# stanFurrer/Robust-Multimodal-Contrastive-Learning

Hardware: AMD Instinct MI355X
Metric: image-text pairs/sec, ViLT-B/32 RMCL step (PGD K=3) (higher is better)
Workload: dtype bf16; 1 GPU; RMCL step, PGD K=3 image attack + MoCo InfoNCE (queue 65536) + full backward + AdamW, ViLT-B/32, bs=64/GPU, 384x384 img + 40 tok (BASELINE configs[2]; [3] when n_gpus=8); global_batch=64, parallelism=dp1, grad_sync=ring/f32, ln_fold=on (shift-robust form)

## Files before the change

robust-multimodal-contrastive-learning_amd/csrc/api.cpp:

```cpp
#include "rmcl_common.h"
#include "kernels.h"
#include "../../include/rmcl.h"
#include <mutex>
#include <string>
#include <unordered_set>

static thread_local std::string g_err;
extern "C" void rmcl_set_error(const char* msg) { g_err = msg ? msg : ""; }

int rmcl_attention_fwd_impl(const void* qkv, const int* mask, void* out, void* probs, float* scores, int B, int N, int H, int dt,
                            int exact, hipStream_t s);
int rmcl_attention_bwd_impl(const void* qkv, const int* mask, const void* probs, const void* dout, const void* out, void* dqkv,
                            float* scores, void* dS, int B, int N, int H, int dt, int exact, hipStream_t s);

#include <vector>
namespace {
struct Prof {
  bool on = false;
  int mask = 0;
  size_t n = 0, cap = 0;
  std::vector<hipEvent_t> ev;
  double flops = 0.0;
} g_prof;
}
// ... 67 lines not shown
  double ms = 0.0;
  for (size_t i = 0; i < g_prof.n; ++i) {
    float t = 0.f;
    HIP_TRY(hipEventSynchronize(g_prof.ev[2 * i + 1]));
    HIP_TRY(hipEventElapsedTime(&t, g_prof.ev[2 * i], g_prof.ev[2 * i + 1]));
    ms += t;
  }
  if (ms_total) *ms_total = ms;
  if (launches) *launches = (int64_t)g_prof.n;
  if (flops_total) *flops_total = g_prof.flops;
  return 0;
}
int rmcl_version(void) { return 1; }

int rmcl_dropout_mask_apply(float* x, int64_t n, uint32_t drop_seed, int layer, int site, float drop_p, void* stream) {
  RMCL_REQUIRE(x && drop_p >= 0.f && drop_p < 1.f, "dropout_mask_apply: bad argument");
  if (drop_p == 0.f) return 0;
  return rmcl_dropout_apply(x, n, rmcl_site_seed(drop_seed, layer, site), (uint32_t)((double)drop_p * 4294967296.0), 1.0f / (1.0f - drop_p),
                            (hipStream_t)stream);
}
extern int g_st_reserve_cus;
extern bool g_attn_fused_bwd;
extern bool g_dw_grouped;
extern int g_attn_fwd_waves;
extern int g_infonce_fold;
extern int g_dp_stagger;
extern int g_attn_bwd_persist;
extern int g_attn_bwd_tpw;
extern int g_gemm_share;
extern bool g_lnfold_centred;
extern int g_prefetch_mask, g_prefetch_wgs;
extern int g_st_res_lds;
extern bool g_preact_tiled;
int rmcl_l2_prefetch_experiment(const void* A, int64_t lda_bytes, int M, int rows_per_tile, int tiles_per_xcd, int col_tiles, const void* B,
                                int64_t ldb_bytes, int nB, int nk, int tick, int lead, int per_xcd, int wgs, int* counter, int64_t* stamps, void* stream) {
  RMCL_REQUIRE(A && B && counter && M > 0 && nk > 0 && per_xcd > 0 && wgs > 0 && col_tiles > 0, "l2_prefetch_experiment: bad argument");
  return rmcl_debug_l2_prefetch(A, (long)lda_bytes, M, rows_per_tile, tiles_per_xcd, col_tiles, B, (long)ldb_bytes, nB, nk, tick, lead, per_xcd, wgs, counter,
                                reinterpret_cast<long long*>(stamps), (hipStream_t)stream);
}
int rmcl_tune_set(int key, int value) {
  if (key == 11) { g_lnfold_centred = value != 0; return 0; }
  if (key == 12) { g_prefetch_mask = value & 7; return 0; }
  if (key == 13) { g_prefetch_wgs = value < 0 ? 0 : (value > 64 ? 64 : value); return 0; }
  if (key == 15) { g_preact_tiled = value != 0; return 0; }
  if (key == 14) { g_st_res_lds = value != 0; return 0; }
  if (key == 7) { g_dp_stagger = value < 0 ? 0 : value; return 0; }
  if (key == 10) { g_gemm_share = value < 1 ? 1 : (value > 8 ? 8 : value); return 0; }
  if (key == 9) { g_attn_bwd_tpw = value; return 0; }
  if (key == 8) { g_attn_bwd_persist = value < 0 ? 0 : value; return 0; }
  if (key == 6) { rmcl_gemm_skinny_set_form(value); return 0; }
  if (key == 0) { rmcl_gemm_fast_set_cfg(value); return 0; }
  if (key == 1) { g_st_reserve_cus = value < 0 ? 0 : (value > 128 ? 128 : value); return 0; }
  if (key == 2) { g_attn_fused_bwd = value != 0; return 0; }
  if (key == 5) { g_infonce_fold = value != 0; return 0; }
  if (key == 4) { g_attn_fwd_waves = value; return 0; }
  if (key == 3) { g_dw_grouped = value != 0; return 0; }
  rmcl_set_error("tune_set: unknown key");
  return -1;
}

int64_t rmcl_heads_stash_bytes(const rmcl_dims* d) { return (int64_t)carve_heads(*d, nullptr, nullptr) + 256; }

int rmcl_heads_forward(const rmcl_dims* d, const float* pool32, const float* head32, const float* xn, void* hstash,
                       float* cls_feats, float* q, void* stream) {
  return rmcl_heads_forward2(d, pool32, head32, xn, hstash, cls_feats, q, 0, stream);
}
int rmcl_heads_forward2(const rmcl_dims* d, const float* pool32, const float* head32, const float* xn, void* hstash,
                        float* cls_feats, float* q, int flags, void* stream) {
  RMCL_REQUIRE(d && pool32 && xn && hstash && cls_feats, "heads_forward: NULL argument");
  RMCL_REQUIRE((flags & ~RMCL_HEADS_NO_WGRAD) == 0, "heads_forward: unknown flag");
  rmcl_layout y;
  rmcl_param_layout(d, &y);
  HeadStash h;
// ... 386 lines not shown
```

robust-multimodal-contrastive-learning_amd/csrc/gemm_sw.hip:

```cpp
#include <type_traits>
#include "rmcl_common.h"
#include "kernels.h"

typedef __bf16 bf16x8 __attribute__((ext_vector_type(8)));
typedef __attribute__((address_space(3))) void lds_void;
typedef const __attribute__((address_space(1))) void glb_void;

#define SW_UNIT 24576
#define SW_BUF (3 * SW_UNIT)
#define SW_LDS (2 * SW_BUF)


#ifdef ST_TRACE
__device__ long long g_sw_trace[2][32];
#define SW_STAMP(i)                                                                                              \
  if (blockIdx.x == 100 && (threadIdx.x & 255) == 0) g_sw_trace[threadIdx.x >> 8][i] = wall_clock64()
extern "C" int rmcl_debug_sw_trace(long long* out) {
  return (int)hipMemcpyFromSymbol(out, HIP_SYMBOL(g_sw_trace), sizeof(long long) * 64);
}
#else
#define SW_STAMP(i)
#endif

template <int N>
__device__ __forceinline__ void sw_wait_vm() {
  asm volatile("s_waitcnt vmcnt(%0)" ::"n"(N) : "memory");
}

__device__ __forceinline__ void sw_stage(const bf16_t* base, const uint32_t (&off)[3], long koff, char* lds_unit, int wave) {
#pragma unroll
  for (int q = 0; q < 3; ++q)
    __builtin_amdgcn_global_load_lds((glb_void*)(base + koff + off[q]), (lds_void*)(lds_unit + (wave * 3 + q) * 1024), 16, 0, 0);
}

__device__ __forceinline__ int sw_gk(int k) { return ((k >> 1) & 1) | (((k >> 3) & 1) << 1); }

template <bool KC>
__device__ __forceinline__ bf16x8 sw_ld(const char* unit, int off, int s) {
  if (KC) {
    return *reinterpret_cast<const bf16x8*>(unit + off);
  } else {
    union { bf16x8 v; s16x4 h[2]; } u;
#pragma unroll
    for (int h = 0; h < 2; ++h)
      u.h[h] = __builtin_amdgcn_ds_read_tr16_b64_v4i16((__attribute__((address_space(3))) s16x4*)(unit + off + s * (32 * 384) + h * (4 * 384)));
    return u.v;
  }
}

#define SW_PHASE_BEGIN()                                  \
  __builtin_amdgcn_sched_barrier(0);                      \
  __builtin_amdgcn_s_barrier();                           \
  asm volatile("s_waitcnt lgkmcnt(0)" ::: "memory");      \
  __builtin_amdgcn_sched_barrier(0);                      \
  __builtin_amdgcn_s_setprio(1)
#define SW_PHASE_END()                                    \
  __builtin_amdgcn_s_setprio(0);                          \
  __builtin_amdgcn_sched_barrier(0);                      \
  __builtin_amdgcn_s_barrier();                           \
  __builtin_amdgcn_sched_barrier(0)

enum { SW_AUX_NONE = 0, SW_AUX_RES = 1, SW_AUX_DGELU = 2, SW_AUX_DGELU_T = 3, SW_AUX_STASH_T = 4 };

struct SWCtx {
  const bf16_t* A;
  const bf16_t* B;
  uint32_t oa[3], ob0[3], ob1[3];
  int aoff[2], boff[2], boffj[3];
  long kstep_b;
  int wave;
};

struct SWAux {
  const bf16_t* aux;
  long ld;
  int m0, n0, M;
};
__device__ __forceinline__ void sw_stage_aux(const SWAux& x, int ch, int unit, char* area, int wave, int lane) {
#pragma unroll
  for (int q = 0; q < 3; ++q) {
    const int L = unit * SW_UNIT + (wave * 3 + q) * 1024 + lane * 16;
    const int r = L / 768, p = (L - r * 768) >> 4;
    const int trow = (r / 48) * 96 + ch * 48 + (r % 48);
    const long m = min(x.m0 + trow, x.M - 1);
    const bf16_t* src = x.aux + m * x.ld + x.n0 + ((p ^ (r & 7)) << 3);
    __builtin_amdgcn_global_load_lds((glb_void*)src, (lds_void*)(area + unit * SW_UNIT + (wave * 3 + q) * 1024), 16, 0, 0);
  }
}

struct SWNoHook { __device__ __forceinline__ void operator()() const {} };
template <bool B_KC, bool LAST, bool AUXST = false, typename HOOK = SWNoHook>
__device__ __forceinline__ void sw_ktile(f32x4 (&acc)[6][6], const SWCtx& c, const char* cur, char* oth, int t1, const SWAux* ax = nullptr, int lane = 0,
                                         const HOOK& hook = HOOK()) {
  bf16x8 a[3][2], b[3][2];
#pragma unroll
  for (int j = 0; j < 3; ++j)
#pragma unroll
    for (int s = 0; s < 2; ++s) b[j][s] = B_KC ? sw_ld<true>(cur + SW_UNIT, j * 2048 + c.boff[s], s) : sw_ld<false>(cur + SW_UNIT, c.boffj[j], s);
#pragma unroll
  for (int i = 0; i < 3; ++i)
#pragma unroll
    for (int s = 0; s < 2; ++s) a[i][s] = sw_ld<true>(cur, i * 2048 + c.aoff[s], s);
  if (!LAST) { sw_stage(c.A, c.oa, (long)t1 * 64, oth, c.wave); sw_wait_vm<3>(); } else { sw_wait_vm<0>(); if (AUXST) sw_stage_aux(*ax, 0, 0, oth, c.wave, lane); hook(); }
  SW_PHASE_BEGIN();
#pragma unroll
  for (int s = 0; s < 2; ++s)
#pragma unroll
    for (int i = 0; i < 3; ++i)
#pragma unroll
      for (int j = 0; j < 3; ++j) acc[i][j] = __builtin_amdgcn_mfma_f32_16x16x32_bf16(b[j][s], a[i][s], acc[i][j], 0, 0, 0);
  SW_PHASE_END();
#pragma unroll
  for (int j = 0; j < 3; ++j)
#pragma unroll
    for (int s = 0; s < 2; ++s) b[j][s] = B_KC ? sw_ld<true>(cur + 2 * SW_UNIT, j * 2048 + c.boff[s], s) : sw_ld<false>(cur + 2 * SW_UNIT, c.boffj[j], s);
  if (!LAST) sw_stage(c.B, c.ob0, (long)t1 * c.kstep_b, oth + SW_UNIT, c.wave);
  else if (AUXST) sw_stage_aux(*ax, 0, 1, oth, c.wave, lane);
  SW_PHASE_BEGIN();
#pragma unroll
  for (int s = 0; s < 2; ++s)
#pragma unroll
    for (int i = 0; i < 3; ++i)
#pragma unroll
      for (int j = 0; j < 3; ++j) acc[i][3 + j] = __builtin_amdgcn_mfma_f32_16x16x32_bf16(b[j][s], a[i][s], acc[i][3 + j], 0, 0, 0);
  SW_PHASE_END();
#pragma unroll
  for (int i = 0; i < 3; ++i)
#pragma unroll
    for (int s = 0; s < 2; ++s) a[i][s] = sw_ld<true>(cur, (3 + i) * 2048 + c.aoff[s], s);
  if (!LAST) sw_stage(c.B, c.ob1, (long)t1 * c.kstep_b, oth + 2 * SW_UNIT, c.wave);
  else if (AUXST) sw_stage_aux(*ax, 0, 2, oth, c.wave, lane);
  SW_PHASE_BEGIN();
#pragma unroll
  for (int s = 0; s < 2; ++s)
#pragma unroll
    for (int i = 0; i < 3; ++i)
#pragma unroll
      for (int j = 0; j < 3; ++j) acc[3 + i][3 + j] = __builtin_amdgcn_mfma_f32_16x16x32_bf16(b[j][s], a[i][s], acc[3 + i][3 + j], 0, 0, 0);
  SW_PHASE_END();
#pragma unroll
  for (int j = 0; j < 3; ++j)
#pragma unroll
    for (int s = 0; s < 2; ++s) b[j][s] = B_KC ? sw_ld<true>(cur + SW_UNIT, j * 2048 + c.boff[s], s) : sw_ld<false>(cur + SW_UNIT, c.boffj[j], s);
  if (!LAST) sw_wait_vm<3>();
  SW_PHASE_BEGIN();
#pragma unroll
  for (int s = 0; s < 2; ++s)
#pragma unroll
    for (int i = 0; i < 3; ++i)
#pragma unroll
      for (int j = 0; j < 3; ++j) acc[3 + i][j] = __builtin_amdgcn_mfma_f32_16x16x32_bf16(b[j][s], a[i][s], acc[3 + i][j], 0, 0, 0);
  SW_PHASE_END();
}

template <bool B_KC, int AUX, typename TO, int LNF = 0, bool DROP = false>
__global__ __launch_bounds__(512) void gemm_sw_kernel(GemmArgs g, int tiles_m, int tiles_n, int rows_per_tile) {
  extern __shared__ __attribute__((aligned(16))) char smem[];
  const int t = threadIdx.x, lane = t & 63;
  const int wave = __builtin_amdgcn_readfirstlane(t >> 6);
  const int wm = wave >> 2, wn = wave & 3;
  SW_STAMP(0);
  const int nwg = tiles_m * tiles_n;
  int bid = blockIdx.x;
  {
    const int xcd = bid & 7, q = nwg >> 3, r = nwg & 7;
    bid = (xcd < r ? xcd * (q + 1) : r * (q + 1) + (xcd - r) * q) + (bid >> 3);
  }
  int tr, tc;
  if (tiles_n % 4 == 0) {
    const int band = bid / (tiles_m * 4), rem = bid - band * (tiles_m * 4);
    tr = rem >> 2;
    tc = band * 4 + (rem & 3);
  } else {
    tr = bid / tiles_n;
    tc = bid - tr * tiles_n;
  }
  const int m0 = tr * rows_per_tile, n0 = tc * 384;
  const int m_end = min(g.M, m0 + rows_per_tile);
  const int nk = g.K / 64;

  SWCtx c;
  c.A = reinterpret_cast<const bf16_t*>(g.A);
  c.B = reinterpret_cast<const bf16_t*>(g.B);
  c.wave = wave;
  c.kstep_b = B_KC ? 64 : 64 * g.ldb;
#pragma unroll
  for (int q = 0; q < 3; ++q) {
    const int row = (wave * 3 + q) * 8 + (lane >> 3);
    const int chunk = (lane & 7) ^ (row & 7);
    const int lin = (wave * 3 + q) * 64 + lane;
    const int k = lin / 24, c16 = (lin - k * 24) ^ (sw_gk(k) << 1);
    c.oa[q] = (uint32_t)min(m0 + row, g.M - 1) * (uint32_t)g.lda + chunk * 8;
    if (B_KC) {
      c.ob0[q] = (uint32_t)(n0 + row) * (uint32_t)g.ldb + chunk * 8;
      c.ob1[q] = (uint32_t)(n0 + 192 + row) * (uint32_t)g.ldb + chunk * 8;
    } else {
      c.ob0[q] = (uint32_t)k * (uint32_t)g.ldb + n0 + c16 * 8;
      c.ob1[q] = c.ob0[q] + 192;
    }
  }
#pragma unroll
  for (int s = 0; s < 2; ++s) {
    const int sw = ((4 * s + (lane >> 4)) ^ (lane & 7)) * 16;
    c.aoff[s] = (wm * 96 + (lane & 15)) * 128 + sw;
    c.boff[s] = (wn * 48 + (lane & 15)) * 128 + sw;
  }
#pragma unroll
  for (int j = 0; j < 3; ++j) {
    const int q = (lane & 15) >> 2, p = lane & 3;
    const int k = 8 * (lane >> 4) + q;
    const int c8 = (wn * 48 + j * 16) / 4 + p;
    c.boffj[j] = k * 384 + (((c8 >> 1) ^ (sw_gk(k) << 1)) * 16) + (c8 & 1) * 8;
  }

  f32x4 acc[6][6];
#pragma unroll
  for (int i = 0; i < 6; ++i)
#pragma unroll
    for (int j = 0; j < 6; ++j) acc[i][j] = f32x4{0.f, 0.f, 0.f, 0.f};

  char* buf0 = smem;
  char* buf1 = smem + SW_BUF;
  float4 pst[LNF == 1 ? 8 : 1];
  float cen = 0.f;
  if constexpr (LNF == 1) {
    if (t < 192) {
      if (n0 == 0 && g.ln_mean && g.ln_center) cen = g.ln_center[min((long)m0 + t, (long)g.M - 1)];
      const float4* pp = reinterpret_cast<const float4*>(g.ln_part + min((long)m0 + t, (long)g.M - 1) * (long)(g.ln_nparts * 2));
      if (g.ln_nparts == 16) {
#pragma unroll
        for (int q = 0; q < 8; ++q) pst[q] = pp[q];
      }
    }
  }
  sw_stage(c.A, c.oa, 0, buf0, wave);
  sw_stage(c.B, c.ob0, 0, buf0 + SW_UNIT, wave);
  sw_stage(c.B, c.ob1, 0, buf0 + 2 * SW_UNIT, wave);
  if constexpr (LNF == 1) {
    if (t < 192) {
      const long m = min((long)m0 + t, (long)g.M - 1);
      float s1 = 0.f, s2 = 0.f;
      if (g.ln_nparts == 16) {
#pragma unroll
        for (int q = 0; q < 8; ++q) { s1 += pst[q].x + pst[q].z; s2 += pst[q].y + pst[q].w; }
      } else {
        const float4* pp = reinterpret_cast<const float4*>(g.ln_part + m * (long)(g.ln_nparts * 2));
        for (int q = 0; q < g.ln_nparts / 2; ++q) { const float4 v = pp[q]; s1 += v.x + v.z; s2 += v.y + v.w; }
      }
      const float inv = 1.0f / (float)g.ln_cols, mean = s1 * inv;
      const float rstd = rsqrtf(fmaxf(s2 * inv - mean * mean, 0.f) + g.ln_eps);
      float* rowstat0 = reinterpret_cast<float*>(smem + SW_LDS);
      rowstat0[2 * t] = mean;
      rowstat0[2 * t + 1] = rstd;
      if (n0 == 0 && g.ln_mean && m0 + t < m_end) { g.ln_mean[m] = mean + cen; g.ln_rstd[m] = rstd; }
    }
    asm volatile("s_waitcnt lgkmcnt(0)" ::: "memory");
  }
  sw_wait_vm<0>();
  __builtin_amdgcn_s_barrier();
  __builtin_amdgcn_sched_barrier(0);
  if (wm == 1) __builtin_amdgcn_s_barrier();
  __builtin_amdgcn_sched_barrier(0);

  SW_STAMP(1);
  int it = 0;
  for (; it + 1 < nk; ++it) {
    char* cur = (it & 1) ? buf1 : buf0;
    char* oth = (it & 1) ? buf0 : buf1;
    sw_ktile<B_KC, false>(acc, c, cur, oth, it + 1);
  }
  constexpr bool AUX_LDS = AUX == SW_AUX_DGELU && sizeof(TO) == 2;
  constexpr bool TILED_DG = AUX == SW_AUX_DGELU_T, TILED_ST = AUX == SW_AUX_STASH_T, DG = AUX == SW_AUX_DGELU || TILED_DG;
  static_assert(!(TILED_DG || TILED_ST) || (sizeof(TO) == 2 && B_KC), "tiled stash: bf16, [cols][K] weights");
  const size_t tblk = (size_t)(tr * tiles_n + tc) * RMCL_PREACT_TILE_ELEMS + rmcl_preact_tiled_off(wave, 0, 0, 0, 0, 0);
  const int tlane = rmcl_preact_tiled_off(0, 0, 0, 0, 0, lane);
  const bf16_t* tl_in = TILED_DG ? reinterpret_cast<const bf16_t*>(g.aux) + tblk : nullptr;
  uint2 tpre[TILED_DG ? 2 : 1][3][3];
  auto tiled_load_row = [&](int GRP, int il) {
    __builtin_amdgcn_sched_barrier(0);
#pragma unroll
    for (int j = 0; j < 3; ++j)
      tpre[TILED_DG && GRP == 3 ? 1 : 0][il][j] = *reinterpret_cast<const uint2*>(tl_in + tlane + rmcl_preact_tiled_off(0, GRP >> 1, GRP & 1, il, j, 0));
    __builtin_amdgcn_sched_barrier(0);
  };
  char* last_cur = (it & 1) ? buf1 : buf0;
  char* aux_area = (it & 1) ? buf0 : buf1;
  SWAux ax{reinterpret_cast<const bf16_t*>(g.aux), (long)g.ld_aux, m0, n0, g.M};
  if constexpr (AUX_LDS) {
    sw_ktile<B_KC, true, true>(acc, c, last_cur, aux_area, 0, &ax, lane);
    sw_wait_vm<0>();
  } else if constexpr (TILED_DG) {
    auto hook = [&]() {
#pragma unroll
      for (int il = 0; il < 3; ++il) tiled_load_row(0, il);
    };
    sw_ktile<B_KC, true, false, decltype(hook)>(acc, c, last_cur, nullptr, 0, nullptr, 0, hook);
  } else {
    sw_ktile<B_KC, true>(acc, c, last_cur, nullptr, 0);
  }
  if (wm == 0) __builtin_amdgcn_s_barrier();
  if constexpr (AUX_LDS) {
    __builtin_amdgcn_s_barrier();
#pragma unroll
    for (int u = 0; u < 3; ++u) sw_stage_aux(ax, 1, u, last_cur, wave, lane);
  }

  SW_STAMP(2);
  const int epi = g.epi;
  TO* C = reinterpret_cast<TO*>(g.C);
  TO* C2 = reinterpret_cast<TO*>(g.C2);
  bf16_t* tl_out = TILED_ST ? reinterpret_cast<bf16_t*>(g.C2) + tblk : nullptr;
  const int mb = m0 + wm * 96 + (lane & 15);
  if constexpr (sizeof(TO) == 2) {
    constexpr int ROWB = 768, PIECES = 48, ROWS = 48, IMG = ROWS * ROWB;
    char* img0 = AUX_LDS ? aux_area + wm * IMG : smem + wm * (2 * IMG);
    const bool stash = !AUX_LDS && (epi & EPI_SAVE_PREACT) != 0;
    float* rowstat = reinterpret_cast<float*>(smem + SW_LDS);
    constexpr bool HOIST = !DG && !DROP;
    float4 bias2[HOIST ? 2 : 1][3], lns2[HOIST ? 2 : 1][LNF == 1 ? 3 : 1];
    if constexpr (HOIST) {
#pragma unroll
      for (int hb = 0; hb < 2; ++hb) {
        const int nbh = n0 + hb * 192 + wn * 48 + 4 * (lane >> 4);
#pragma unroll
        for (int j = 0; j < 3; ++j) {
          if constexpr (LNF == 1) {
            bias2[hb][j] = *reinterpret_cast<const float4*>(g.ln_c + nbh + j * 16);
            lns2[hb][j] = *reinterpret_cast<const float4*>(g.ln_s + nbh + j * 16);
          } else {
            bias2[hb][j] = (epi & EPI_BIAS) ? *reinterpret_cast<const float4*>(g.bias + nbh + j * 16) : make_float4(0.f, 0.f, 0.f, 0.f);
          }
        }
      }
    }
    float2 rs6[LNF == 1 ? 6 : 1];
    if constexpr (LNF == 1) {
#pragma unroll
      for (int i = 0; i < 6; ++i) rs6[i] = *reinterpret_cast<const float2*>(rowstat + 2 * (wm * 96 + i * 16 + (lane & 15)));
    }
    int woff[2][3];
#pragma unroll
    for (int hb = 0; hb < 2; ++hb)
#pragma unroll
      for (int j = 0; j < 3; ++j) {
        const int r = lane & 15, e8 = hb * 48 + wn * 12 + j * 4 + (lane >> 4);
        woff[hb][j] = r * ROWB + (((e8 >> 1) ^ (r & 7)) * 16) + (e8 & 1) * 8;
        asm volatile("" : "+v"(woff[hb][j]));
      }
    int rb_row[3], rb_lds[3];
    uint32_t rb_dst[3];
    {
      const int tg = (wave & 3) * 64 + lane, row0 = tg / PIECES, cp0 = tg - row0 * PIECES;
#pragma unroll
      for (int kk = 0; kk < 3; ++kk) {
        const int t16 = cp0 + 16 * kk, wrap = t16 >= PIECES ? 1 : 0, cp = t16 - wrap * PIECES, row = row0 + 5 * kk + wrap;
        rb_row[kk] = row;
        rb_lds[kk] = row * ROWB + cp * 16;
        rb_dst[kk] = (uint32_t)row * (uint32_t)g.ldc + (uint32_t)((cp ^ (row & 7)) * 8);
        asm volatile("" : "+v"(rb_row[kk]), "+v"(rb_lds[kk]), "+v"(rb_dst[kk]));
      }
    }
    const uint32_t dbase_aux = DROP ? (uint32_t)mb * (uint32_t)g.ld_aux : 0u, dbase_c = DROP ? (uint32_t)mb * (uint32_t)g.ldc : 0u;
    auto chunk_loop = [&](auto gelu_c, auto stash_c, auto dm_c) {
      constexpr bool GELU = decltype(gelu_c)::value, STASH = decltype(stash_c)::value;
      constexpr int DM = decltype(dm_c)::value;
#pragma unroll
      for (int ch = 0; ch < 2; ++ch) {
        char* aux_ch = ch == 0 ? aux_area : last_cur;
        char* img = AUX_LDS ? aux_ch + wm * IMG : img0;
// ... 31 lines not shown
              }
            }
          }
#pragma unroll
          for (int il = 0; il < 3; ++il) {
            const int i = ch * 3 + il;
            float mean_m = 0.f, rstd_m = 1.f;
            if constexpr (LNF == 1) { mean_m = rs6[i].x; rstd_m = rs6[i].y; }
#pragma unroll
            for (int j = 0; j < 3; ++j) {
              const f32x4 av = acc[i][hb * 3 + j], bv = f4v(bias[j]);
              f32x4 v;
              if constexpr (LNF == 1) v = rstd_m * (av - mean_m * f4v(lns[j])) + bv;
              else v = g.alpha * av + bv;
              if constexpr (TILED_DG) v *= gelu_poly_grad4(bf2f4(tpre[TILED_DG && ch * 2 + hb == 3 ? 1 : 0][il][j]));
              else if (AUX == SW_AUX_DGELU) v *= gelu_poly_grad4(bf2f4(pre[il][j]));
              if constexpr (DROP && (DM & 2) != 0) {
                if (DM == 2 || (epi & EPI_DROP_BWD)) {
                  const uint32_t di = dbase_aux + (uint32_t)(i * 16) * (uint32_t)g.ld_aux + (uint32_t)(nb + j * 16);
                  drop_scale4(g.drop_seed, di, g.drop_thresh, g.drop_inv_keep, v);
                }
              }
              const int off = woff[hb][j] + il * 16 * ROWB;
              if constexpr (STASH && TILED_ST) *reinterpret_cast<uint2*>(tl_out + tlane + rmcl_preact_tiled_off(0, ch, hb, il, j, 0)) = f2bf4(v);
              else if constexpr (STASH) *reinterpret_cast<uint2*>(img + IMG + off) = f2bf4(v);
              if constexpr (GELU) v = gelu_poly4(v);
              if constexpr (DROP && (DM & 1) != 0) {
                if (DM == 1 || (epi & EPI_DROPOUT)) {
                  const uint32_t ci = dbase_c + (uint32_t)(i * 16) * (uint32_t)g.ldc + (uint32_t)(nb + j * 16);
                  drop_scale4(g.drop_seed, ci, g.drop_thresh, g.drop_inv_keep, v);
                }
              }
              const uint2 pk = f2bf4(v);
              *reinterpret_cast<uint2*>(img + off) = pk;
            }
            if constexpr (TILED_DG) {
              if (ch * 2 + hb < 2) tiled_load_row(ch * 2 + hb + 1, il);
              if (ch * 2 + hb == 1 && il == 2) {
#pragma unroll
                for (int l3 = 0; l3 < 3; ++l3) tiled_load_row(3, l3);
              }
            }
          }
        }
        SW_STAMP(4 + 3 * ch);
        __builtin_amdgcn_s_barrier();
        {
          const int mrow = m0 + wm * 96 + ch * ROWS, lim = m_end - mrow;
          const uint32_t cbase = (uint32_t)mrow * (uint32_t)g.ldc + (uint32_t)n0;
#pragma unroll
          for (int t3 = 0; t3 < 3; ++t3)
#pragma unroll
            for (int kk = 0; kk < 3; ++kk) {
              if (rb_row[kk] + 16 * t3 < lim) {
                const size_t dst = (size_t)(cbase + (uint32_t)(16 * t3) * (uint32_t)g.ldc + rb_dst[kk]);
                *reinterpret_cast<float4*>(C + dst) = *reinterpret_cast<const float4*>(img + rb_lds[kk] + t3 * 16 * ROWB);
                if constexpr (STASH && !TILED_ST) *reinterpret_cast<float4*>(C2 + dst) = *reinterpret_cast<const float4*>(img + IMG + rb_lds[kk] + t3 * 16 * ROWB);
              }
            }
        }
        if constexpr (AUX_LDS) {
          if (ch == 0) { if (m0 + 144 <= m_end) sw_wait_vm<9>(); else sw_wait_vm<0>(); }
        }
        SW_STAMP(5 + 3 * ch);
        __builtin_amdgcn_s_barrier();
        SW_STAMP(6 + 3 * ch);
      }
    };
    {
      using T1 = std::integral_constant<bool, true>;
      using T0 = std::integral_constant<bool, false>;
      using D0 = std::integral_constant<int, 0>;
      using D1 = std::integral_constant<int, 1>;
      using D2 = std::integral_constant<int, 2>;
      using D3 = std::integral_constant<int, 3>;
      const bool gelu = (epi & EPI_GELU) != 0;
      const int dm = DROP ? (((epi & EPI_DROPOUT) ? 1 : 0) | ((epi & EPI_DROP_BWD) ? 2 : 0)) : 0;
      if constexpr (TILED_ST) {
        if constexpr (DROP) chunk_loop(T1{}, T1{}, D1{}); else chunk_loop(T1{}, T1{}, D0{});
      } else if constexpr (TILED_DG) {
        if constexpr (DROP) chunk_loop(T0{}, T0{}, D2{}); else chunk_loop(T0{}, T0{}, D0{});
      } else if constexpr (!DROP) {
        if constexpr (AUX_LDS) {
          if (gelu) chunk_loop(T1{}, T0{}, D0{}); else chunk_loop(T0{}, T0{}, D0{});
        } else {
          if (gelu && stash) chunk_loop(T1{}, T1{}, D0{});
          else if (gelu) chunk_loop(T1{}, T0{}, D0{});
          else if (stash) chunk_loop(T0{}, T1{}, D0{});
          else chunk_loop(T0{}, T0{}, D0{});
        }
      } else if constexpr (AUX_LDS) {
        if (!gelu && dm == 2) chunk_loop(T0{}, T0{}, D2{});
        else if (gelu) chunk_loop(T1{}, T0{}, D3{});
        else chunk_loop(T0{}, T0{}, D3{});
      } else {
        if (gelu && stash && dm == 1) chunk_loop(T1{}, T1{}, D1{});
        else if (gelu && !stash && dm == 1) chunk_loop(T1{}, T0{}, D1{});
        else if (gelu && stash) chunk_loop(T1{}, T1{}, D3{});
        else if (gelu) chunk_loop(T1{}, T0{}, D3{});
        else if (stash) chunk_loop(T0{}, T1{}, D3{});
        else chunk_loop(T0{}, T0{}, D3{});
      }
    }
  } else {
#pragma unroll
    for (int hb = 0; hb < 2; ++hb) {
      const int nb = n0 + hb * 192 + wn * 48 + 4 * (lane >> 4);
      float4 bias[3];
#pragma unroll
      for (int j = 0; j < 3; ++j) bias[j] = (epi & EPI_BIAS) ? *reinterpret_cast<const float4*>(g.bias + nb + j * 16) : make_float4(0.f, 0.f, 0.f, 0.f);
      uint2 pre[AUX == SW_AUX_DGELU ? 6 : 1][3];
#pragma unroll
      for (int i = 0; i < 6; ++i) {
        const long mr = min(mb + i * 16, g.M - 1);
#pragma unroll
        for (int j = 0; j < 3; ++j)
          if (AUX == SW_AUX_DGELU) pre[i][j] = *reinterpret_cast<const uint2*>(reinterpret_cast<const bf16_t*>(g.aux) + mr * g.ld_aux + nb + j * 16);
      }
#pragma unroll
      for (int i = 0; i < 6; ++i) {
        const int m = mb + i * 16;
        const bool live = m < m_end;
#pragma unroll
        for (int j = 0; j < 3; ++j) {
          const f32x4 av = acc[i][hb * 3 + j];
          float v[4] = {g.alpha * av[0] + bias[j].x, g.alpha * av[1] + bias[j].y, g.alpha * av[2] + bias[j].z, g.alpha * av[3] + bias[j].w};
          if (AUX == SW_AUX_DGELU) {
            const uint2 u = pre[i][j];
            v[0] *= gelu_poly_grad(__uint_as_float(u.x << 16)); v[1] *= gelu_poly_grad(__uint_as_float(u.x & 0xffff0000u));
            v[2] *= gelu_poly_grad(__uint_as_float(u.y << 16)); v[3] *= gelu_poly_grad(__uint_as_float(u.y & 0xffff0000u));
          }
          const long ci = (long)m * g.ldc + nb + j * 16;
          if ((epi & EPI_SAVE_PREACT) && live) store4<TO>(C2 + ci, v);
          if (epi & EPI_GELU) {
#pragma unroll
            for (int r = 0; r < 4; ++r) v[r] = gelu_poly(v[r]);
          }
          if (live) store4<TO>(C + ci, v);
        }
      }
    }
  }
#ifdef ST_TRACE
  SW_STAMP(10);
  asm volatile("s_waitcnt vmcnt(0)" ::: "memory");
  SW_STAMP(11);
#endif
}

bool rmcl_gemm_sw_supported(const GemmArgs& g, int a_kc, int b_kc) {
  if (!a_kc || g.nb1 > 1 || g.nb2 > 1 || g.splitk > 1) return false;
  if (g.N % 384 != 0 || g.K % 64 != 0 || g.K < 128) return false;
  if ((long)g.M * g.lda >= (1L << 31) || (long)(b_kc ? g.N : g.K) * g.ldb >= (1L << 31)) return false;
  if ((long)g.M * g.ldc >= (1L << 31)) return false;
  if (g.epi & ~(EPI_BIAS | EPI_GELU | EPI_SAVE_PREACT | EPI_DGELU | EPI_LNFOLD | EPI_DROPOUT | EPI_DROP_BWD | EPI_PREACT_TILED)) return false;
  if ((g.epi & EPI_DROP_BWD) && !(g.epi & EPI_DGELU)) return false;
  if ((g.epi & EPI_PREACT_TILED) && (!b_kc || !(g.epi & EPI_SAVE_PREACT) == !(g.epi & EPI_DGELU))) return false;
  if ((g.epi & EPI_PREACT_TILED) && (g.epi & EPI_SAVE_PREACT) && !(g.epi & EPI_GELU)) return false;
  if ((g.epi & EPI_PREACT_TILED) && (g.epi & EPI_DGELU) && (g.epi & (EPI_BIAS | EPI_GELU | EPI_DROPOUT))) return false;
  if (g.epi & EPI_LNFOLD) {
    if (!b_kc || (g.epi & (EPI_BIAS | EPI_DGELU)) || !g.ln_s || !g.ln_c || !g.ln_part || g.ln_nparts % 2 || g.ln_nparts <= 0 || g.ln_cols <= 0) return false;
  }
  return true;
}

double rmcl_gemm_sw_fill(const GemmArgs& g, int cus) {
  const long tiles = (long)cdiv(g.M, 192) * (g.N / 384);
  return (double)tiles / (double)(cdiv(tiles, (long)cus) * cus);
}

template <bool B_KC, int AUX, typename TO, bool DROP = false>
static int launch_sw3(const GemmArgs& g, hipStream_t s) {
  static RmclLdsOnce once;
  RMCL_TRY(rmcl_set_max_lds(once, reinterpret_cast<const void*>(gemm_sw_kernel<B_KC, AUX, TO, 0, DROP>), SW_LDS));
  const int tm = cdiv(g.M, 192), tn = g.N / 384, rows = cdiv(g.M, tm);
  RMCL_LAUNCH((gemm_sw_kernel<B_KC, AUX, TO, 0, DROP>), dim3(tm * tn), dim3(512), SW_LDS, s, g, tm, tn, rows);
  RMCL_CHECK_LAUNCH();
  return 0;
}

template <bool B_KC, int AUX>
static int launch_sw2(const GemmArgs& g, int dt_out, hipStream_t s) {
  if (g.epi & (EPI_DROPOUT | EPI_DROP_BWD)) {
    RMCL_REQUIRE(dt_out == RMCL_BF16, "gemm_sw: the dropout epilogues write bf16");
    return launch_sw3<B_KC, AUX, bf16_t, true>(g, s);
  }
  return dt_out == RMCL_F32 ? launch_sw3<B_KC, AUX, float>(g, s) : launch_sw3<B_KC, AUX, bf16_t>(g, s);
}

template <bool B_KC>
static int launch_sw(const GemmArgs& g, int dt_out, hipStream_t s) {
  if (g.epi & EPI_PREACT_TILED) {
    if constexpr (B_KC) {
      RMCL_REQUIRE(dt_out == RMCL_BF16, "gemm_sw: the tiled pre-activation stash is bf16");
      const bool drop = (g.epi & (EPI_DROPOUT | EPI_DROP_BWD)) != 0;
      if (g.epi & EPI_DGELU) return drop ? launch_sw3<true, SW_AUX_DGELU_T, bf16_t, true>(g, s) : launch_sw3<true, SW_AUX_DGELU_T, bf16_t>(g, s);
      return drop ? launch_sw3<true, SW_AUX_STASH_T, bf16_t, true>(g, s) : launch_sw3<true, SW_AUX_STASH_T, bf16_t>(g, s);
    } else {
      RMCL_REQUIRE(false, "gemm_sw: the tiled pre-activation stash needs [cols][K] weights");
    }
  }
  if (g.epi & EPI_DGELU) return launch_sw2<B_KC, SW_AUX_DGELU>(g, dt_out, s);
  return launch_sw2<B_KC, SW_AUX_NONE>(g, dt_out, s);
}

template <bool DROP, int AUX = SW_AUX_NONE>
static int launch_sw_lnf(const GemmArgs& g, hipStream_t s) {
  constexpr int LDS = SW_LDS + 2048;
  static RmclLdsOnce once;
  RMCL_TRY(rmcl_set_max_lds(once, reinterpret_cast<const void*>((gemm_sw_kernel<true, AUX, bf16_t, 1, DROP>)), LDS));
  const int tm = cdiv(g.M, 192), tn = g.N / 384, rows = cdiv(g.M, tm);
  RMCL_LAUNCH((gemm_sw_kernel<true, AUX, bf16_t, 1, DROP>), dim3(tm * tn), dim3(512), LDS, s, g, tm, tn, rows);
  RMCL_CHECK_LAUNCH();
  return 0;
}

int rmcl_launch_gemm_sw(const GemmArgs& g, int dt_out, int b_kc, hipStream_t s) {
  if (g.epi & EPI_LNFOLD) {
    RMCL_REQUIRE(b_kc && dt_out == RMCL_BF16, "gemm_sw: the LayerNorm-folded form is [rows][K] x [cols][K] with bf16 output");
    if (g.epi & EPI_PREACT_TILED) return (g.epi & EPI_DROPOUT) ? launch_sw_lnf<true, SW_AUX_STASH_T>(g, s) : launch_sw_lnf<false, SW_AUX_STASH_T>(g, s);
    return (g.epi & EPI_DROPOUT) ? launch_sw_lnf<true>(g, s) : launch_sw_lnf<false>(g, s);
  }
  return b_kc ? launch_sw<true>(g, dt_out, s) : launch_sw<false>(g, dt_out, s);
}
```

Before: 2043 pairs/s.

## Add persistent grid form to software-pipelined GEMM with next-tile prefetch

Adds a persistent variant of the 192x384 software-pipelined GEMM kernel that launches about one workgroup per CU and loops over tiles. It prefetches the next tile's A/B k-tile into LDS during the current tile's epilogue, which removes per-tile launch and ramp-up cost and tail waste when tiles exceed CUs. It is on by default whenever the tile count exceeds the CU cap, and can be turned off through a tune key. In exchange the epilogue staging image moves into the second buffer, and there are more LDS hazards and inline asm waits to keep correct.

```diff
diff --git a/robust-multimodal-contrastive-learning_amd/csrc/api.cpp b/robust-multimodal-contrastive-learning_amd/csrc/api.cpp
--- a/robust-multimodal-contrastive-learning_amd/csrc/api.cpp
+++ b/robust-multimodal-contrastive-learning_amd/csrc/api.cpp
@@ -123,6 +123,7 @@
 extern int g_prefetch_mask, g_prefetch_wgs;
 extern int g_st_res_lds;
 extern bool g_preact_tiled;
+extern int g_sw_persist;
 int rmcl_l2_prefetch_experiment(const void* A, int64_t lda_bytes, int M, int rows_per_tile, int tiles_per_xcd, int col_tiles, const void* B,
                                 int64_t ldb_bytes, int nB, int nk, int tick, int lead, int per_xcd, int wgs, int* counter, int64_t* stamps, void* stream) {
   RMCL_REQUIRE(A && B && counter && M > 0 && nk > 0 && per_xcd > 0 && wgs > 0 && col_tiles > 0, "l2_prefetch_experiment: bad argument");
@@ -130,6 +131,7 @@
                                 reinterpret_cast<long long*>(stamps), (hipStream_t)stream);
 }
 int rmcl_tune_set(int key, int value) {
+  if (key == 16) { g_sw_persist = value < 0 ? -1 : (value > 4096 ? 4096 : value); return 0; }
   if (key == 11) { g_lnfold_centred = value != 0; return 0; }
   if (key == 12) { g_prefetch_mask = value & 7; return 0; }
   if (key == 13) { g_prefetch_wgs = value < 0 ? 0 : (value > 64 ? 64 : value); return 0; }
diff --git a/robust-multimodal-contrastive-learning_amd/csrc/gemm_sw.hip b/robust-multimodal-contrastive-learning_amd/csrc/gemm_sw.hip
--- a/robust-multimodal-contrastive-learning_amd/csrc/gemm_sw.hip
+++ b/robust-multimodal-contrastive-learning_amd/csrc/gemm_sw.hip
@@ -14,7 +14,7 @@
 #ifdef ST_TRACE
 __device__ long long g_sw_trace[2][32];
 #define SW_STAMP(i)                                                                                              \
-  if (blockIdx.x == 100 && (threadIdx.x & 255) == 0) g_sw_trace[threadIdx.x >> 8][i] = wall_clock64()
+  if (blockIdx.x == 100 && (threadIdx.x & 255) == 0) g_sw_trace[threadIdx.x >> 8][(i) + sw_stamp_base] = wall_clock64()
 extern "C" int rmcl_debug_sw_trace(long long* out) {
   return (int)hipMemcpyFromSymbol(out, HIP_SYMBOL(g_sw_trace), sizeof(long long) * 64);
 }
@@ -31,6 +31,22 @@
 #pragma unroll
   for (int q = 0; q < 3; ++q)
     __builtin_amdgcn_global_load_lds((glb_void*)(base + koff + off[q]), (lds_void*)(lds_unit + (wave * 3 + q) * 1024), 16, 0, 0);
+}
+
+typedef uint32_t u32x2 __attribute__((ext_vector_type(2)));
+__device__ __forceinline__ void sw_lds_write64(uint32_t a, uint2 v) {
+  const u32x2 w = {v.x, v.y};
+  asm volatile("ds_write_b64 %0, %1" : : "v"(a), "v"(w) : "memory");
+}
+__device__ __forceinline__ f32x4 sw_lds_read128(uint32_t a) {
+  f32x4 v;
+  asm volatile("ds_read_b128 %0, %1" : "=v"(v) : "v"(a) : "memory");
+  return v;
+}
+__device__ __forceinline__ u32x2 sw_lds_read64(uint32_t a) {
+  u32x2 v;
+  asm volatile("ds_read_b64 %0, %1" : "=v"(v) : "v"(a) : "memory");
+  return v;
 }
 
 __device__ __forceinline__ int sw_gk(int k) { return ((k >> 1) & 1) | (((k >> 3) & 1) << 1); }
@@ -65,6 +81,7 @@
 struct SWCtx {
   const bf16_t* A;
   const bf16_t* B;
+  const bf16_t* B1;
   uint32_t oa[3], ob0[3], ob1[3];
   int aoff[2], boff[2], boffj[3];
   long kstep_b;
@@ -89,9 +106,9 @@
 }
 
 struct SWNoHook { __device__ __forceinline__ void operator()() const {} };
-template <bool B_KC, bool LAST, bool AUXST = false, typename HOOK = SWNoHook>
+template <bool B_KC, bool LAST, bool AUXST = false, typename HOOK = SWNoHook, bool PERS = false>
 __device__ __forceinline__ void sw_ktile(f32x4 (&acc)[6][6], const SWCtx& c, const char* cur, char* oth, int t1, const SWAux* ax = nullptr, int lane = 0,
-                                         const HOOK& hook = HOOK()) {
+                                         const HOOK& hook = HOOK(), bool nxt = false, bool nowait = false) {
   bf16x8 a[3][2], b[3][2];
 #pragma unroll
   for (int j = 0; j < 3; ++j)
@@ -101,7 +118,15 @@
   for (int i = 0; i < 3; ++i)
 #pragma unroll
     for (int s = 0; s < 2; ++s) a[i][s] = sw_ld<true>(cur, i * 2048 + c.aoff[s], s);
-  if (!LAST) { sw_stage(c.A, c.oa, (long)t1 * 64, oth, c.wave); sw_wait_vm<3>(); } else { sw_wait_vm<0>(); if (AUXST) sw_stage_aux(*ax, 0, 0, oth, c.wave, lane); hook(); }
+  if (!LAST) {
+    sw_stage(c.A, c.oa, (long)t1 * 64, oth, c.wave);
+    if (PERS) { if (!nowait) sw_wait_vm<3>(); } else sw_wait_vm<3>();
+  } else {
+    sw_wait_vm<0>();
+    if (AUXST) sw_stage_aux(*ax, 0, 0, oth, c.wave, lane);
+    hook();
+    if (PERS) { if (nxt) sw_stage(c.A, c.oa, 0, oth, c.wave); }
+  }
   SW_PHASE_BEGIN();
 #pragma unroll
   for (int s = 0; s < 2; ++s)
@@ -116,6 +141,7 @@
     for (int s = 0; s < 2; ++s) b[j][s] = B_KC ? sw_ld<true>(cur + 2 * SW_UNIT, j * 2048 + c.boff[s], s) : sw_ld<false>(cur + 2 * SW_UNIT, c.boffj[j], s);
   if (!LAST) sw_stage(c.B, c.ob0, (long)t1 * c.kstep_b, oth + SW_UNIT, c.wave);
   else if (AUXST) sw_stage_aux(*ax, 0, 1, oth, c.wave, lane);
+  else if (PERS) { if (nxt) sw_stage(c.B, c.ob0, 0, oth + SW_UNIT, c.wave); }
   SW_PHASE_BEGIN();
 #pragma unroll
   for (int s = 0; s < 2; ++s)
@@ -128,8 +154,9 @@
   for (int i = 0; i < 3; ++i)
 #pragma unroll
     for (int s = 0; s < 2; ++s) a[i][s] = sw_ld<true>(cur, (3 + i) * 2048 + c.aoff[s], s);
-  if (!LAST) sw_stage(c.B, c.ob1, (long)t1 * c.kstep_b, oth + 2 * SW_UNIT, c.wave);
+  if (!LAST) { if (PERS) sw_stage(c.B1, c.ob0, (long)t1 * c.kstep_b, oth + 2 * SW_UNIT, c.wave); else sw_stage(c.B, c.ob1, (long)t1 * c.kstep_b, oth + 2 * SW_UNIT, c.wave); }
   else if (AUXST) sw_stage_aux(*ax, 0, 2, oth, c.wave, lane);
+  else if (PERS) { if (nxt) sw_stage(c.B1, c.ob0, 0, oth + 2 * SW_UNIT, c.wave); }
   SW_PHASE_BEGIN();
 #pragma unroll
   for (int s = 0; s < 2; ++s)
@@ -153,19 +180,32 @@
   SW_PHASE_END();
 }
 
-template <bool B_KC, int AUX, typename TO, int LNF = 0, bool DROP = false>
-__global__ __launch_bounds__(512) void gemm_sw_kernel(GemmArgs g, int tiles_m, int tiles_n, int rows_per_tile) {
+template <bool B_KC, int AUX, typename TO, int LNF, bool DROP, bool PERS>
+__device__ __forceinline__ void sw_body(GemmArgs g, int tiles_m, int tiles_n, int rows_per_tile) {
+  static_assert(!PERS || (B_KC && sizeof(TO) == 2 && (AUX == SW_AUX_NONE || AUX == SW_AUX_DGELU_T || AUX == SW_AUX_STASH_T)), "persistent form: one LDS image per group");
   extern __shared__ __attribute__((aligned(16))) char smem[];
-  const int t = threadIdx.x, lane = t & 63;
+  const int t = threadIdx.x, lane0 = t & 63;
   const int wave = __builtin_amdgcn_readfirstlane(t >> 6);
   const int wm = wave >> 2, wn = wave & 3;
+  [[maybe_unused]] int sw_stamp_base = 0;
   SW_STAMP(0);
-  const int nwg = tiles_m * tiles_n;
+  const int ntiles = tiles_m * tiles_n;
+  const int nwg = PERS ? (int)gridDim.x : ntiles;
   int bid = blockIdx.x;
   {
     const int xcd = bid & 7, q = nwg >> 3, r = nwg & 7;
     bid = (xcd < r ? xcd * (q + 1) : r * (q + 1) + (xcd - r) * q) + (bid >> 3);
   }
+  auto tile_rc = [&](int id, int& r_, int& c_) {
+    if (tiles_n % 4 == 0) {
+      const int band = id / (tiles_m * 4), rem = id - band * (tiles_m * 4);
+      r_ = rem >> 2;
+      c_ = band * 4 + (rem & 3);
+    } else {
+      r_ = id / tiles_n;
+      c_ = id - r_ * tiles_n;
+    }
+  };
   int tr, tc;
   if (tiles_n % 4 == 0) {
     const int band = bid / (tiles_m * 4), rem = bid - band * (tiles_m * 4);
@@ -175,20 +215,39 @@
     tr = bid / tiles_n;
     tc = bid - tr * tiles_n;
   }
-  const int m0 = tr * rows_per_tile, n0 = tc * 384;
-  const int m_end = min(g.M, m0 + rows_per_tile);
+  int m0 = tr * rows_per_tile, n0 = tc * 384;
+  int m_end = min(g.M, m0 + rows_per_tile);
   const int nk = g.K / 64;
 
   SWCtx c;
   c.A = reinterpret_cast<const bf16_t*>(g.A);
   c.B = reinterpret_cast<const bf16_t*>(g.B);
+  c.B1 = c.B + (PERS ? (size_t)192 * (size_t)g.ldb : 0);
   c.wave = wave;
   c.kstep_b = B_KC ? 64 : 64 * g.ldb;
+  int ln = lane0;
+  auto set_offsets = [&](int m0_, int n0_) {
+#pragma unroll
+    for (int q = 0; q < 3; ++q) {
+      const int row = (wave * 3 + q) * 8 + (ln >> 3);
+      const int chunk = (ln & 7) ^ (row & 7);
+      const int lin = (wave * 3 + q) * 64 + ln;
+      const int k = lin / 24, c16 = (lin - k * 24) ^ (sw_gk(k) << 1);
+      c.oa[q] = (uint32_t)min(m0_ + row, g.M - 1) * (uint32_t)g.lda + chunk * 8;
+      if (B_KC) {
+        c.ob0[q] = (uint32_t)(n0_ + row) * (uint32_t)g.ldb + chunk * 8;
+        if (!PERS) c.ob1[q] = (uint32_t)(n0_ + 192 + row) * (uint32_t)g.ldb + chunk * 8;
+      } else {
+        c.ob0[q] = (uint32_t)k * (uint32_t)g.ldb + n0_ + c16 * 8;
+        c.ob1[q] = c.ob0[q] + 192;
+      }
+    }
+  };
 #pragma unroll
   for (int q = 0; q < 3; ++q) {
-    const int row = (wave * 3 + q) * 8 + (lane >> 3);
-    const int chunk = (lane & 7) ^ (row & 7);
-    const int lin = (wave * 3 + q) * 64 + lane;
+    const int row = (wave * 3 + q) * 8 + (lane0 >> 3);
+    const int chunk = (lane0 & 7) ^ (row & 7);
+    const int lin = (wave * 3 + q) * 64 + lane0;
     const int k = lin / 24, c16 = (lin - k * 24) ^ (sw_gk(k) << 1);
     c.oa[q] = (uint32_t)min(m0 + row, g.M - 1) * (uint32_t)g.lda + chunk * 8;
     if (B_KC) {
@@ -199,16 +258,31 @@
       c.ob1[q] = c.ob0[q] + 192;
     }
   }
+  auto set_frag_offsets = [&]() {
+#pragma unroll
+    for (int s = 0; s < 2; ++s) {
+      const int sw = ((4 * s + (ln >> 4)) ^ (ln & 7)) * 16;
+      c.aoff[s] = (wm * 96 + (ln & 15)) * 128 + sw;
+      c.boff[s] = (wn * 48 + (ln & 15)) * 128 + sw;
+    }
+#pragma unroll
+    for (int j = 0; j < 3; ++j) {
+      const int q = (ln & 15) >> 2, p = ln & 3;
+      const int k = 8 * (ln >> 4) + q;
+      const int c8 = (wn * 48 + j * 16) / 4 + p;
+      c.boffj[j] = k * 384 + (((c8 >> 1) ^ (sw_gk(k) << 1)) * 16) + (c8 & 1) * 8;
+    }
+  };
 #pragma unroll
   for (int s = 0; s < 2; ++s) {
-    const int sw = ((4 * s + (lane >> 4)) ^ (lane & 7)) * 16;
-    c.aoff[s] = (wm * 96 + (lane & 15)) * 128 + sw;
-    c.boff[s] = (wn * 48 + (lane & 15)) * 128 + sw;
+    const int sw = ((4 * s + (lane0 >> 4)) ^ (lane0 & 7)) * 16;
+    c.aoff[s] = (wm * 96 + (lane0 & 15)) * 128 + sw;
+    c.boff[s] = (wn * 48 + (lane0 & 15)) * 128 + sw;
   }
 #pragma unroll
   for (int j = 0; j < 3; ++j) {
-    const int q = (lane & 15) >> 2, p = lane & 3;
-    const int k = 8 * (lane >> 4) + q;
+    const int q = (lane0 & 15) >> 2, p = lane0 & 3;
+    const int k = 8 * (lane0 >> 4) + q;
     const int c8 = (wn * 48 + j * 16) / 4 + p;
     c.boffj[j] = k * 384 + (((c8 >> 1) ^ (sw_gk(k) << 1)) * 16) + (c8 & 1) * 8;
   }
@@ -223,7 +297,7 @@
   char* buf1 = smem + SW_BUF;
   float4 pst[LNF == 1 ? 8 : 1];
   float cen = 0.f;
-  if constexpr (LNF == 1) {
+  auto ln_fetch = [&]() {
     if (t < 192) {
       if (n0 == 0 && g.ln_mean && g.ln_center) cen = g.ln_center[min((long)m0 + t, (long)g.M - 1)];
       const float4* pp = reinterpret_cast<const float4*>(g.ln_part + min((long)m0 + t, (long)g.M - 1) * (long)(g.ln_nparts * 2));
@@ -232,15 +306,12 @@
         for (int q = 0; q < 8; ++q) pst[q] = pp[q];
       }
     }
-  }
-  sw_stage(c.A, c.oa, 0, buf0, wave);
-  sw_stage(c.B, c.ob0, 0, buf0 + SW_UNIT, wave);
-  sw_stage(c.B, c.ob1, 0, buf0 + 2 * SW_UNIT, wave);
-  if constexpr (LNF == 1) {
+  };
+  auto ln_finish = [&](auto pre_c) {
     if (t < 192) {
       const long m = min((long)m0 + t, (long)g.M - 1);
       float s1 = 0.f, s2 = 0.f;
-      if (g.ln_nparts == 16) {
+      if (decltype(pre_c)::value && g.ln_nparts == 16) {
 #pragma unroll
         for (int q = 0; q < 8; ++q) { s1 += pst[q].x + pst[q].z; s2 += pst[q].y + pst[q].w; }
       } else {
@@ -255,19 +326,47 @@
       if (n0 == 0 && g.ln_mean && m0 + t < m_end) { g.ln_mean[m] = mean + cen; g.ln_rstd[m] = rstd; }
     }
     asm volatile("s_waitcnt lgkmcnt(0)" ::: "memory");
-  }
+  };
+  if constexpr (LNF == 1) ln_fetch();
+  sw_stage(c.A, c.oa, 0, buf0, wave);
+  sw_stage(c.B, c.ob0, 0, buf0 + SW_UNIT, wave);
+  if constexpr (PERS) sw_stage(c.B1, c.ob0, 0, buf0 + 2 * SW_UNIT, wave);
+  else sw_stage(c.B, c.ob1, 0, buf0 + 2 * SW_UNIT, wave);
+  if constexpr (LNF == 1) ln_finish(std::integral_constant<bool, true>{});
   sw_wait_vm<0>();
   __builtin_amdgcn_s_barrier();
   __builtin_amdgcn_sched_barrier(0);
+  [[maybe_unused]] int tile = bid;
+  [[maybe_unused]] bool later = false;
+  for (;;) {
+  int lane = lane0;
+  if constexpr (PERS) { asm volatile("" : "+v"(lane)); ln = lane; }
   if (wm == 1) __builtin_amdgcn_s_barrier();
   __builtin_amdgcn_sched_barrier(0);
 
   SW_STAMP(1);
   int it = 0;
-  for (; it + 1 < nk; ++it) {
-    char* cur = (it & 1) ? buf1 : buf0;
-    char* oth = (it & 1) ? buf0 : buf1;
-    sw_ktile<B_KC, false>(acc, c, cur, oth, it + 1);
+  if constexpr (PERS) {
+    for (; it + 1 < nk; ++it) {
+      char* cur = (it & 1) ? buf1 : buf0;
+      char* oth = (it & 1) ? buf0 : buf1;
+      sw_ktile<B_KC, false, false, SWNoHook, true>(acc, c, cur, oth, it + 1, nullptr, 0, SWNoHook(), false, later && it == 0);
+    }
+  } else {
+    for (; it + 1 < nk; ++it) {
+      char* cur = (it & 1) ? buf1 : buf0;
+      char* oth = (it & 1) ? buf0 : buf1;
+      sw_ktile<B_KC, false>(acc, c, cur, oth, it + 1);
+    }
+  }
+  [[maybe_unused]] int ntr = tr, ntc = tc;
+  [[maybe_unused]] bool has_next = false;
+  if constexpr (PERS) {
+    has_next = tile + nwg < ntiles;
+    if (has_next) {
+      tile_rc(tile + nwg, ntr, ntc);
+      set_offsets(ntr * rows_per_tile, ntc * 384);
+    }
   }
   constexpr bool AUX_LDS = AUX == SW_AUX_DGELU && sizeof(TO) == 2;
   constexpr bool TILED_DG = AUX == SW_AUX_DGELU_T, TILED_ST = AUX == SW_AUX_STASH_T, DG = AUX == SW_AUX_DGELU || TILED_DG;
@@ -294,11 +393,21 @@
 #pragma unroll
       for (int il = 0; il < 3; ++il) tiled_load_row(0, il);
     };
-    sw_ktile<B_KC, true, false, decltype(hook)>(acc, c, last_cur, nullptr, 0, nullptr, 0, hook);
+    if constexpr (PERS) sw_ktile<B_KC, true, false, decltype(hook), true>(acc, c, last_cur, buf0, 0, nullptr, 0, hook, last_cur != buf0);
+    else sw_ktile<B_KC, true, false, decltype(hook)>(acc, c, last_cur, nullptr, 0, nullptr, 0, hook);
   } else {
-    sw_ktile<B_KC, true>(acc, c, last_cur, nullptr, 0);
+    if constexpr (PERS) sw_ktile<B_KC, true, false, SWNoHook, true>(acc, c, last_cur, buf0, 0, nullptr, 0, SWNoHook(), last_cur != buf0);
+    else sw_ktile<B_KC, true>(acc, c, last_cur, nullptr, 0);
   }
   if (wm == 0) __builtin_amdgcn_s_barrier();
+  if constexpr (PERS) {
+    if (last_cur == buf0) {
+      sw_stage(c.A, c.oa, 0, buf0, wave);
+      sw_stage(c.B, c.ob0, 0, buf0 + SW_UNIT, wave);
+      sw_stage(c.B1, c.ob0, 0, buf0 + 2 * SW_UNIT, wave);
+    }
+    __builtin_amdgcn_s_waitcnt(0xC07F);
+  }
   if constexpr (AUX_LDS) {
     __builtin_amdgcn_s_barrier();
 #pragma unroll
@@ -313,7 +422,8 @@
   const int mb = m0 + wm * 96 + (lane & 15);
   if constexpr (sizeof(TO) == 2) {
     constexpr int ROWB = 768, PIECES = 48, ROWS = 48, IMG = ROWS * ROWB;
-    char* img0 = AUX_LDS ? aux_area + wm * IMG : smem + wm * (2 * IMG);
+    char* img0 = AUX_LDS ? aux_area + wm * IMG : PERS ? buf1 + wm * IMG : smem + wm * (2 * IMG);
+    [[maybe_unused]] const uint32_t img_a = lds_addr(img0);
     const bool stash = !AUX_LDS && (epi & EPI_SAVE_PREACT) != 0;
     float* rowstat = reinterpret_cast<float*>(smem + SW_LDS);
     constexpr bool HOIST = !DG && !DROP;
@@ -334,7 +444,14 @@
       }
     }
     float2 rs6[LNF == 1 ? 6 : 1];
-    if constexpr (LNF == 1) {
+    if constexpr (LNF == 1 && PERS) {
+      u32x2 rsu[6];
+#pragma unroll
+      for (int i = 0; i < 6; ++i) rsu[i] = sw_lds_read64(lds_addr(rowstat) + 8 * (wm * 96 + i * 16 + (lane & 15)));
+      asm volatile("s_waitcnt lgkmcnt(0)" : "+v"(rsu[0]), "+v"(rsu[1]), "+v"(rsu[2]), "+v"(rsu[3]), "+v"(rsu[4]), "+v"(rsu[5]) : : "memory");
+#pragma unroll
+      for (int i = 0; i < 6; ++i) rs6[i] = make_float2(__uint_as_float(rsu[i].x), __uint_as_float(rsu[i].y));
+    } else if constexpr (LNF == 1) {
 #pragma unroll
       for (int i = 0; i < 6; ++i) rs6[i] = *reinterpret_cast<const float2*>(rowstat + 2 * (wm * 96 + i * 16 + (lane & 15)));
     }
@@ -432,7 +549,8 @@
                 }
               }
               const uint2 pk = f2bf4(v);
-              *reinterpret_cast<uint2*>(img + off) = pk;
+              if constexpr (PERS) sw_lds_write64(img_a + (uint32_t)off, pk);
+              else *reinterpret_cast<uint2*>(img + off) = pk;
             }
             if constexpr (TILED_DG) {
               if (ch * 2 + hb < 2) tiled_load_row(ch * 2 + hb + 1, il);
@@ -444,8 +562,38 @@
           }
         }
         SW_STAMP(4 + 3 * ch);
+        if constexpr (PERS) {
+          static_assert(!PERS || !STASH || TILED_ST, "persistent form: no row-major stash image");
+          if (ch == 0) sw_wait_vm<(TILED_DG || TILED_ST) ? 18 : 0>();
+          asm volatile("s_waitcnt lgkmcnt(0)" ::: "memory");
+        }
         __builtin_amdgcn_s_barrier();
-        {
+        if constexpr (PERS) {
+          const int mrow = m0 + wm * 96 + ch * ROWS, lim = m_end - mrow;
+          const uint32_t cbase = (uint32_t)mrow * (uint32_t)g.ldc + (uint32_t)n0;
+          f32x4 w[2][3];
+#pragma unroll
+          for (int kk = 0; kk < 3; ++kk) w[0][kk] = sw_lds_read128(img_a + (uint32_t)rb_lds[kk]);
+#pragma unroll
+          for (int t3 = 0; t3 < 3; ++t3) {
+            f32x4(&wc)[3] = w[t3 & 1];
+            if (t3 < 2) {
+              f32x4(&wn2)[3] = w[(t3 + 1) & 1];
+#pragma unroll
+              for (int kk = 0; kk < 3; ++kk) wn2[kk] = sw_lds_read128(img_a + (uint32_t)(rb_lds[kk] + (t3 + 1) * 16 * ROWB));
+              asm volatile("s_waitcnt lgkmcnt(3)" : "+v"(wc[0]), "+v"(wc[1]), "+v"(wc[2]) : : "memory");
+            } else {
+              asm volatile("s_waitcnt lgkmcnt(0)" : "+v"(wc[0]), "+v"(wc[1]), "+v"(wc[2]) : : "memory");
+            }
+#pragma unroll
+            for (int kk = 0; kk < 3; ++kk) {
+              if (rb_row[kk] + 16 * t3 < lim) {
+                const size_t dst = (size_t)(cbase + (uint32_t)(16 * t3) * (uint32_t)g.ldc + rb_dst[kk]);
+                *reinterpret_cast<f32x4*>(C + dst) = wc[kk];
+              }
+            }
+          }
+        } else {
           const int mrow = m0 + wm * 96 + ch * ROWS, lim = m_end - mrow;
           const uint32_t cbase = (uint32_t)mrow * (uint32_t)g.ldc + (uint32_t)n0;
 #pragma unroll
@@ -480,6 +628,16 @@
         if constexpr (DROP) chunk_loop(T1{}, T1{}, D1{}); else chunk_loop(T1{}, T1{}, D0{});
       } else if constexpr (TILED_DG) {
         if constexpr (DROP) chunk_loop(T0{}, T0{}, D2{}); else chunk_loop(T0{}, T0{}, D0{});
+      } else if constexpr (PERS && LNF == 1) {
+        if constexpr (DROP) chunk_loop(T1{}, T0{}, D1{}); else chunk_loop(T1{}, T0{}, D0{});
+      } else if constexpr (PERS) {
+        if constexpr (!DROP) {
+          if (gelu) chunk_loop(T1{}, T0{}, D0{}); else chunk_loop(T0{}, T0{}, D0{});
+        } else {
+          if (gelu && dm == 1) chunk_loop(T1{}, T0{}, D1{});
+          else if (gelu) chunk_loop(T1{}, T0{}, D3{});
+          else chunk_loop(T0{}, T0{}, D3{});
+        }
       } else if constexpr (!DROP) {
         if constexpr (AUX_LDS) {
           if (gelu) chunk_loop(T1{}, T0{}, D0{}); else chunk_loop(T0{}, T0{}, D0{});
@@ -541,11 +699,51 @@
       }
     }
   }
+  if constexpr (!PERS) {
+    break;
+  } else {
+    if (!has_next) break;
+    SW_STAMP(10);
+    tile += nwg;
+    m0 = ntr * rows_per_tile;
+    n0 = ntc * 384;
+    m_end = min(g.M, m0 + rows_per_tile);
+    if constexpr (LNF == 1) {
+      if (ntr != tr) {
+        if (t < 192 && n0 == 0 && g.ln_mean && g.ln_center) cen = g.ln_center[min((long)m0 + t, (long)g.M - 1)];
+        ln_finish(std::integral_constant<bool, false>{});
+        __builtin_amdgcn_s_barrier();
+      }
+    }
+    tr = ntr;
+    tc = ntc;
+    later = true;
+    set_offsets(m0, n0);
+    set_frag_offsets();
+#pragma unroll
+    for (int i = 0; i < 6; ++i)
+#pragma unroll
+      for (int j = 0; j < 6; ++j) acc[i][j] = f32x4{0.f, 0.f, 0.f, 0.f};
+#ifdef ST_TRACE
+    sw_stamp_base = 12;
+#endif
+  }
+  }
 #ifdef ST_TRACE
   SW_STAMP(10);
   asm volatile("s_waitcnt vmcnt(0)" ::: "memory");
   SW_STAMP(11);
 #endif
+}
+
+template <bool B_KC, int AUX, typename TO, int LNF = 0, bool DROP = false>
+__global__ __launch_bounds__(512) void gemm_sw_kernel(GemmArgs g, int tiles_m, int tiles_n, int rows_per_tile) {
+  sw_body<B_KC, AUX, TO, LNF, DROP, false>(g, tiles_m, tiles_n, rows_per_tile);
+}
+
+template <int AUX, int LNF, bool DROP>
+__global__ __launch_bounds__(512) void gemm_swp_kernel(GemmArgs g, int tiles_m, int tiles_n, int rows_per_tile) {
+  sw_body<true, AUX, bf16_t, LNF, DROP, true>(g, tiles_m, tiles_n, rows_per_tile);
 }
 
 bool rmcl_gemm_sw_supported(const GemmArgs& g, int a_kc, int b_kc) {
@@ -569,11 +767,44 @@
   return (double)tiles / (double)(cdiv(tiles, (long)cus) * cus);
 }
 
+int g_sw_persist = -1;
+extern int g_st_reserve_cus;
+
+static int sw_num_cus() {
+  static int n = 0;
+  if (!n) {
+    int dev = 0;
+    if (hipGetDevice(&dev) != hipSuccess || hipDeviceGetAttribute(&n, hipDeviceAttributeMultiprocessorCount, dev) != hipSuccess || n <= 0) n = 256;
+  }
+  return n;
+}
+
+static int sw_persist_grid(int tiles) {
+  if (g_sw_persist == 0) return 0;
+  const int cap = g_sw_persist > 0 ? g_sw_persist : max(8, sw_num_cus() - g_st_reserve_cus);
+  return cap < tiles ? cap : 0;
+}
+
+template <bool B_KC, int AUX, typename TO>
+constexpr bool sw_persist_form() {
+  return B_KC && sizeof(TO) == 2 && (AUX == SW_AUX_NONE || AUX == SW_AUX_DGELU_T || AUX == SW_AUX_STASH_T);
+}
+
 template <bool B_KC, int AUX, typename TO, bool DROP = false>
 static int launch_sw3(const GemmArgs& g, hipStream_t s) {
+  const int tm = cdiv(g.M, 192), tn = g.N / 384, rows = cdiv(g.M, tm);
+  if constexpr (sw_persist_form<B_KC, AUX, TO>()) {
+    const int grid = (AUX == SW_AUX_NONE && (g.epi & EPI_SAVE_PREACT)) ? 0 : sw_persist_grid(tm * tn);
+    if (grid > 0) {
+      static RmclLdsOnce once_p;
+      RMCL_TRY(rmcl_set_max_lds(once_p, reinterpret_cast<const void*>(gemm_swp_kernel<AUX, 0, DROP>), SW_LDS));
+      RMCL_LAUNCH((gemm_swp_kernel<AUX, 0, DROP>), dim3(grid), dim3(512), SW_LDS, s, g, tm, tn, rows);
+      RMCL_CHECK_LAUNCH();
+      return 0;
+    }
+  }
   static RmclLdsOnce once;
   RMCL_TRY(rmcl_set_max_lds(once, reinterpret_cast<const void*>(gemm_sw_kernel<B_KC, AUX, TO, 0, DROP>), SW_LDS));
-  const int tm = cdiv(g.M, 192), tn = g.N / 384, rows = cdiv(g.M, tm);
   RMCL_LAUNCH((gemm_sw_kernel<B_KC, AUX, TO, 0, DROP>), dim3(tm * tn), dim3(512), SW_LDS, s, g, tm, tn, rows);
   RMCL_CHECK_LAUNCH();
   return 0;
@@ -607,9 +838,18 @@
 template <bool DROP, int AUX = SW_AUX_NONE>
 static int launch_sw_lnf(const GemmArgs& g, hipStream_t s) {
   constexpr int LDS = SW_LDS + 2048;
+  const int tm = cdiv(g.M, 192), tn = g.N / 384, rows = cdiv(g.M, tm);
+  const bool fc1_epi = (g.epi & EPI_GELU) && !(g.epi & EPI_SAVE_PREACT) && (!DROP || (g.epi & EPI_DROPOUT));
+  const int grid = (AUX == SW_AUX_NONE && !fc1_epi) ? 0 : sw_persist_grid(tm * tn);
+  if (grid > 0) {
+    static RmclLdsOnce once_p;
+    RMCL_TRY(rmcl_set_max_lds(once_p, reinterpret_cast<const void*>((gemm_swp_kernel<AUX, 1, DROP>)), LDS));
+    RMCL_LAUNCH((gemm_swp_kernel<AUX, 1, DROP>), dim3(grid), dim3(512), LDS, s, g, tm, tn, rows);
+    RMCL_CHECK_LAUNCH();
+    return 0;
+  }
   static RmclLdsOnce once;
   RMCL_TRY(rmcl_set_max_lds(once, reinterpret_cast<const void*>((gemm_sw_kernel<true, AUX, bf16_t, 1, DROP>)), LDS));
-  const int tm = cdiv(g.M, 192), tn = g.N / 384, rows = cdiv(g.M, tm);
   RMCL_LAUNCH((gemm_sw_kernel<true, AUX, bf16_t, 1, DROP>), dim3(tm * tn), dim3(512), LDS, s, g, tm, tn, rows);
   RMCL_CHECK_LAUNCH();
   return 0;
```

Result: no change. 2043 pairs/s (-0.0%).
